# lightbulb128/troy

Measured on AMD Instinct MI355X. Metric: ct x ct multiply+relinearize ops/sec, BFV N=2^15 L=14; achieved HBM GB/s vs peak, higher is better.
Workload: dtype u64; 1 GPU; bfv_n32768_l14; scheme=BFV, N=32768, K=15, L=14, batch_per_gpu=256, parallelism=batch-shard x1, streams_per_gpu=2, Bsk=15, limb_transforms_per_op=443

## Files before the change

### troy_amd/csrc/device_types.h

```cpp
#pragma once
#include "modarith.h"

namespace troyhip {

struct PrimeDesc {
    u64 p, cr0, cr1, two_p;
    Shoup inv_n;
    Shoup iroot_last_scaled;
    Shoup r64;
    const Shoup *root;
    const Shoup *iroot;
    Shoup aux;
    const Shoup *root_fp;
    const Shoup *iroot_fp;
    Shoup inv_n_fp, iroot_last_scaled_fp;
    const u64 *root_w;
    const u64 *iroot_w;
};
__host__ __device__ inline Mod mod_of(const PrimeDesc &d) { return Mod{d.p, d.cr0, d.cr1}; }

struct LimbMap {
    uint8_t id[64];
    uint32_t period, inner;
    uint64_t lean;
    uint64_t fp;
    const uint64_t *host_primes;
};

#define TROY_BUF_OOB 0x80000000u
#ifdef TROYHIP_CPU_EMUL
#define TROY_WAVE_SYNC() hip_emul::park(2)
#define TROY_DYN_LDS(type, name) static type name[160 * 1024 / sizeof(type)]
#define TROY_GLDS16(gptr, lds_base) memcpy((char *)(lds_base) + 16 * (threadIdx.x & 63), (const void *)(gptr), 16)
#define TROY_GLDS16_POL(gptr, lds_base, pol) TROY_GLDS16(gptr, lds_base)
struct MfmaFrag { int8_t bytes[16]; };
struct MfmaAcc { int32_t v[16]; };
#define TROY_MFMA_I8(fa, fb, fc) hip_emul::mfma_i32_32x32x32_i8((fa).bytes, (fb).bytes, (fc).v)
inline void frag_set_word(MfmaFrag &f, int pos, u64 v) { memcpy(f.bytes + 8 * pos, &v, 8); }
struct BufRsrc { char *base; u32 bytes; };
inline BufRsrc make_rsrc(const void *p, u32 bytes) { return BufRsrc{(char *)p, bytes}; }
inline u64 buf_load_u64(BufRsrc r, u32 off) { u64 v = 0; if ((u64)off + 8 <= r.bytes) memcpy(&v, r.base + off, 8); return v; }
inline void buf_store_u64(BufRsrc r, u32 off, u64 v) { if ((u64)off + 8 <= r.bytes) memcpy(r.base + off, &v, 8); }
#define TROY_WAIT_VMEM() hip_emul::park(2)
#define TROY_WAIT_LDS() hip_emul::park(2)
#else
struct MfmaFrag { int bytes __attribute__((ext_vector_type(4))); };
struct MfmaAcc { int v __attribute__((ext_vector_type(16))); };
#define TROY_MFMA_I8(fa, fb, fc) ((fc).v = __builtin_amdgcn_mfma_i32_32x32x32_i8((fa).bytes, (fb).bytes, (fc).v, 0, 0, 0))
__device__ __forceinline__ void frag_set_word(MfmaFrag &f, int pos, u64 v) {
    f.bytes[2 * pos] = (int)(u32)v;
    f.bytes[2 * pos + 1] = (int)(u32)(v >> 32);
}
typedef __amdgpu_buffer_rsrc_t BufRsrc;
typedef unsigned int troy_v2u __attribute__((ext_vector_type(2)));
__device__ __forceinline__ BufRsrc make_rsrc(const void *p, u32 bytes) { return __builtin_amdgcn_make_buffer_rsrc((void *)p, 0, (int)bytes, 0x00020000); }
__device__ __forceinline__ u64 buf_load_u64(BufRsrc r, u32 off) {
    const troy_v2u v = __builtin_amdgcn_raw_buffer_load_b64(r, (int)off, 0, 0);
    return (u64)v.x | ((u64)v.y << 32);
}
__device__ __forceinline__ void buf_store_u64(BufRsrc r, u32 off, u64 v) {
    troy_v2u d;
    d.x = (u32)v;
    d.y = (u32)(v >> 32);
    __builtin_amdgcn_raw_buffer_store_b64(d, r, (int)off, 0, 0);
}
#define TROY_GLDS16(gptr, lds_base)                                                                                      \
    __builtin_amdgcn_global_load_lds((const __attribute__((address_space(1))) void *)(gptr), (__attribute__((address_space(3))) void *)(lds_base), 16, 0, 0)
#define TROY_GLDS16_POL(gptr, lds_base, pol)                                                                             \
    __builtin_amdgcn_global_load_lds((const __attribute__((address_space(1))) void *)(gptr), (__attribute__((address_space(3))) void *)(lds_base), 16, 0, pol)
#define TROY_WAIT_VMEM() asm volatile("s_waitcnt vmcnt(0)" ::: "memory")
#define TROY_WAIT_LDS() asm volatile("s_waitcnt lgkmcnt(0)" ::: "memory")
#define TROY_WAVE_SYNC() __builtin_amdgcn_wave_barrier()
#define TROY_DYN_LDS(type, name) extern __shared__ __attribute__((aligned(16))) type name[]
#endif

}
```

### troy_amd/csrc/ntt2.hip

```cpp
#include "kernels.h"
#include "bfly.h"
#include "fpmod.h"
#include <cstdio>
#include <cstdlib>
#include <cstring>
#include <type_traits>

namespace troyhip {

#define N2_THREADS 256
#define N2_LOGT 11
#define N2_T 2048

struct Ntt2Args {
    u64 *data;
    const u64 *src;
    u64 src_ostride;
    const PrimeDesc *primes;
    LimbMap map;
    int logn;
    unsigned tiles_per_row_log;
    unsigned m_total;
    unsigned rows_per_wg;
    unsigned chunks;
// ... 127 lines not shown
            for (int st = 0; st < R; st++) {
                const int dist = 1 << st, off = (1 << R) - ((1 << R) >> st);
                const bool last = STRIDED && (LS + st == NS - 1);
#pragma unroll
                for (int u = 0; u < G; u++)
#pragma unroll
                    for (int blk = 0; blk < ((1 << R) >> (st + 1)); blk++)
#pragma unroll
                        for (int k = 0; k < dist; k++) {
                            const int ix = (u << R) + blk * 2 * dist + k, iy = ix + dist;
                            const Shoup &w = tw[u][off + blk];
                            const double X = fp_of_bits(x[ix]), Y = fp_of_bits(x[iy]);
                            const double sum = X + Y, dif = X - Y;
                            x[ix] = fp_bits(last ? fp_mulmod_wp(sum, fp_of_bits(inv_n.op), fp_of_bits(inv_n.quo), fc) : sum);
                            x[iy] = fp_bits(fp_mulmod_wp(dif, fp_of_bits(w.op), fp_of_bits(w.quo), fc));
                        }
            }
            return;
        }
#pragma unroll
        for (int st = 0; st < R; st++) {
#pragma unroll
            for (int u = 0; u < G; u++) {
                const int half = (1 << R) >> (st + 1);
#pragma unroll
                for (int blk = 0; blk < (1 << st); blk++)
#pragma unroll
                    for (int k = 0; k < half; k++) {
                        const int ix = (u << R) + blk * 2 * half + k, iy = ix + half;
                        const Shoup &w = tw[u][(1 << st) - 1 + blk];
                        const double X = fp_of_bits(x[ix]);
                        const double v = fp_mulmod_wp(fp_of_bits(x[iy]), fp_of_bits(w.op), fp_of_bits(w.quo), fc);
                        x[ix] = fp_bits(X + v);
                        x[iy] = fp_bits(X - v);
                    }
            }
        }
    }
    __device__ static __forceinline__ void compute(u64 (&x)[8], const Shoup (&tw)[G][NTW], const PrimeDesc &pd, const bool lean = false) {
        const PrimeConst pc = make_prime_const(pd.p);
#pragma unroll
        for (int st = 0; st < R; st++) {
            u64 X[4], Y[4];
            Shoup w[4];
            int ix[4], iy[4];
            int n = 0;
#pragma unroll
            for (int u = 0; u < G; u++) {
                if (!INV) {
                    const int half = (1 << R) >> (st + 1);
#pragma unroll
                    for (int blk = 0; blk < (1 << st); blk++)
#pragma unroll
                        for (int k = 0; k < half; k++) {
                            ix[n] = (u << R) + blk * 2 * half + k;
                            iy[n] = ix[n] + half;
                            w[n] = tw[u][(1 << st) - 1 + blk];
                            n++;
                        }
                } else {
                    const int dist = 1 << st;
                    const int off = (1 << R) - ((1 << R) >> st);
#pragma unroll
                    for (int blk = 0; blk < ((1 << R) >> (st + 1)); blk++)
#pragma unroll
                        for (int k = 0; k < dist; k++) {
                            ix[n] = (u << R) + blk * 2 * dist + k;
                            iy[n] = ix[n] + dist;
                            w[n] = tw[u][off + blk];
                            n++;
                        }
                }
            }
#pragma unroll
            for (int i = 0; i < 4; i++) { X[i] = x[ix[i]]; Y[i] = x[iy[i]]; }
            if (!INV) {
                if (lean) ct_bfly4_ng<UNIFORM>(X, Y, w, pc); else ct_bfly4<UNIFORM>(X, Y, w, pc);
            } else if (STRIDED && (LS + st == NS - 1)) gs_bfly4_last<UNIFORM>(X, Y, w, pd.inv_n, pc);
            else gs_bfly4<UNIFORM>(X, Y, w, pc);
#pragma unroll
            for (int i = 0; i < 4; i++) { x[ix[i]] = X[i]; x[iy[i]] = Y[i]; }
        }
    }
    __device__ static __forceinline__ void lds_read(u64 (&x)[8], const u64 *lds, const unsigned t) {
#pragma unroll
        for (int u = 0; u < G; u++)
#pragma unroll
            for (int e = 0; e < (1 << R); e++) x[(u << R) + e] = lds[swz(elem(t + THREADS * u, e))];
    }
    __device__ static __forceinline__ void lds_write(const u64 (&x)[8], u64 *lds, const unsigned t) {
#pragma unroll
        for (int u = 0; u < G; u++)
#pragma unroll
            for (int e = 0; e < (1 << R); e++) lds[swz(elem(t + THREADS * u, e))] = x[(u << R) + e];
    }
    __device__ static __forceinline__ unsigned unit_perm(unsigned lane) { return 4 * (lane & 15) + (lane >> 4); }
    __device__ static __forceinline__ void stage_issue(const u64 *row, unsigned tile, u64 *wave_stage) {
        static_assert(!STRIDED && NS == 9 && R == 3 && LS == 0, "staging is defined for the first round of the contiguous pass");
        const unsigned lane = threadIdx.x & 63, w = threadIdx.x >> 6;
        const u64 *src = row + ((size_t)tile << N2_LOGT) + 512 * w + 2 * (INV ? unit_perm(lane) : lane);
#pragma unroll
        for (int i = 0; i < 4; i++) TROY_GLDS16_POL(src + 128 * i, wave_stage + 128 * i, 2);
    }
    __device__ static __forceinline__ void stage_read(u64 (&x)[8], const u64 *wave_stage) {
        const unsigned lane = threadIdx.x & 63;
        if (INV) {
            const u64 *mine = wave_stage + 128 * (lane >> 4) + 2 * (lane & 15);
#pragma unroll
            for (int j = 0; j < 4; j++) {
                const ulonglong2 v = *reinterpret_cast<const ulonglong2 *>(mine + 32 * j);
                x[2 * j] = v.x;
                x[2 * j + 1] = v.y;
            }
        } else {
#pragma unroll
            for (int e = 0; e < 8; e++) x[e] = wave_stage[lane + 64 * e];
        }
    }
    __device__ static __forceinline__ void store_via_lds(const u64 (&x)[8], u64 *row, unsigned tile, u64 *wave_xchg) {
        const unsigned lane = threadIdx.x & 63, w = threadIdx.x >> 6;
        u64 *mine = wave_xchg + 128 * (lane >> 4) + 2 * (lane & 15);
#pragma unroll
        for (int j = 0; j < 4; j++) {
            ulonglong2 v;
            v.x = x[2 * j];
            v.y = x[2 * j + 1];
            *reinterpret_cast<ulonglong2 *>(mine + 32 * j) = v;
        }
        TROY_WAVE_SYNC();
        u64 *dst = row + ((size_t)tile << N2_LOGT) + 512 * w + 2 * unit_perm(lane);
#pragma unroll
        for (int c = 0; c < 4; c++) {
            const ulonglong2 v = *reinterpret_cast<const ulonglong2 *>(wave_xchg + 128 * c + 2 * lane);
            *reinterpret_cast<ulonglong2 *>(dst + 128 * c) = v;
        }
    }
    __device__ static __forceinline__ void tensor_epilogue(u64 (&x)[8], u64 (&tx)[3][8], unsigned mm, u64 *out, unsigned period, unsigned slot, unsigned tile, int logn,
                                                           const Mod &m, u64 *xchg, const bool lean, const FpPrime *fc = nullptr) {
        const PrimeConst pc = make_prime_const(m.p);
        if (fc) {
#pragma unroll
            for (int e = 0; e < 8; e++) x[e] = fp_canonical(fp_of_bits(x[e]), *fc, m.p);
        } else if (lean) {
#pragma unroll
            for (int h = 0; h < 2; h++) {
                u64 v[4] = {x[4 * h], x[4 * h + 1], x[4 * h + 2], x[4 * h + 3]};
                lite_reduce4(v, (u32)m.cr1, pc);
#pragma unroll
                for (int i = 0; i < 4; i++) x[4 * h + i] = v[i];
            }
        } else {
#pragma unroll
            for (int h = 0; h < 2; h++) {
                u64 v[4] = {x[4 * h], x[4 * h + 1], x[4 * h + 2], x[4 * h + 3]};
                reduce4_from_8p(v, pc);
#pragma unroll
                for (int i = 0; i < 4; i++) x[4 * h + i] = v[i];
            }
        }
        const unsigned vr = mm & 3;
        if (vr < 3) {
#pragma unroll
            for (int i = 0; i < 3; i++)
                if ((int)vr == i) {
#pragma unroll
                    for (int e = 0; e < 8; e++) tx[i][e] = x[e];
                }
            return;
        }
        const unsigned b = mm >> 2;
        const ProdMod pm = make_prod_mod(m);
        u64 d[3][8];
#pragma unroll
        for (int e = 0; e < 8; e++) {
            const u64 a0 = tx[0][e], a1 = tx[1][e], b0 = tx[2][e], b1 = x[e];
            d[0][e] = reduce_prod((u128)a0 * b0, pm);
            d[1][e] = reduce_prod((u128)a0 * b1 + (u128)a1 * b0, pm);
// ... 72 lines not shown
                    v.x = x[(u << R) + e];
                    v.y = x[(u << R) + e + 1];
                    *reinterpret_cast<ulonglong2 *>(row + g_index<STRIDED, NS, LOGC>(tile, elem(q, e), logn)) = v;
                }
            } else {
#pragma unroll
                for (int e = 0; e < (1 << R); e++) n2_st<STRIDED && !INV>(row + g_index<STRIDED, NS, LOGC>(tile, elem(q, e), logn), x[(u << R) + e]);
            }
        }
    }
    template <int FINAL> __device__ static __forceinline__ void md_write(u64 (&x)[8], const Ntt2Args &a, unsigned o, unsigned slot, unsigned tile, int logn, const Mod &m,
                                                                         const PrimeDesc &pd, const FpPrime *fc = nullptr) {
        static_assert(INV && STRIDED && G == 1, "the mod-down epilogue belongs to the last inverse pass");
        const u64 p = m.p;
        const PrimeConst pc = make_prime_const(p);
        const u64 *sp = a.data + (((u64)o * a.map.period + a.md_dl) << logn);
        u64 *ct = a.md_ct + (u64)(o >> 1) * a.md_ct_bstride + (((u64)(o & 1) * a.md_dl + slot) << logn);
        const u64 *base = a.md_base ? a.md_base + (u64)(o >> 1) * a.md_base_bstride + (((u64)(o & 1) * a.md_dl + slot) << logn) : ct;
        const bool from_zero = a.md_base && (o & 1) && a.md_base_polys < 2;
        const ulonglong2 *sh = reinterpret_cast<const ulonglong2 *>(a.md_share) + ((u64)o << logn);
        const u64 c_p = FINAL == 3 ? barrett64(a.md_half, m) : 0;
#pragma unroll
        for (int h = 0; h < 2; h++) {
            u64 v[4] = {x[4 * h], x[4 * h + 1], x[4 * h + 2], x[4 * h + 3]};
            if (fc) {
#pragma unroll
                for (int i = 0; i < 4; i++) v[i] = fp_canonical(fp_of_bits(v[i]), *fc, p);
            } else {
                reduce4_from_4p(v, pc);
            }
            u64 al[4], ah[4], c[4];
            unsigned n[4];
#pragma unroll
            for (int i = 0; i < 4; i++) {
                n[i] = g_index<STRIDED, NS, LOGC>(tile, elem(threadIdx.x, 4 * h + i), logn);
                if (FINAL == 3) { al[i] = sp[n[i]]; ah[i] = 0; }
                else { const ulonglong2 t = sh[n[i]]; al[i] = t.x; ah[i] = t.y; }
                c[i] = from_zero ? 0 : base[n[i]];
            }
#pragma unroll
            for (int i = 0; i < 4; i++) {
                u64 w;
                if (FINAL == 3) {
                    u64 tl = al[i] + a.md_half;
                    tl = tl >= a.md_qk ? tl - a.md_qk : tl;
                    w = p + c_p - barrett64(tl, m);
                } else {
                    w = p - barrett128(al[i], ah[i], m);
                }
                u64 r = v[i] + mul_shoup(w, pd.aux, p);
                r = r >= p ? r - p : r;
                ct[n[i]] = addmod(c[i], r, p);
            }
        }
    }
};

template <int NS> struct Plan;
template <> struct Plan<3> { static constexpr int r[4] = {3, 0, 0, 0}; };
template <> struct Plan<4> { static constexpr int r[4] = {3, 1, 0, 0}; };
template <> struct Plan<5> { static constexpr int r[4] = {3, 2, 0, 0}; };
template <> struct Plan<6> { static constexpr int r[4] = {3, 3, 0, 0}; };
template <> struct Plan<7> { static constexpr int r[4] = {3, 1, 3, 0}; };
template <> struct Plan<9> { static constexpr int r[4] = {3, 3, 3, 0}; };
template <> struct Plan<10> { static constexpr int r[4] = {3, 3, 3, 1}; };
template <> struct Plan<11> { static constexpr int r[4] = {3, 3, 3, 2}; };

template <int INV, int STRIDED, int NS, int LOGC, int FINAL, int REDUCE, int MAC, int FP>
__device__ __forceinline__ void ntt2_body(const Ntt2Args &a) {
    static_assert(!FP || !(INV && MAC), "FP64 instances: every pass of the two-pass transform and its fusions");
    constexpr int LOGT = STRIDED ? NS + LOGC : N2_LOGT;
    __shared__ u64 lds[2][1 << LOGT];
    using P = Plan<NS>;
    constexpr bool WAVE_PRIVATE = !STRIDED && NS == 9;
    constexpr bool KS = MAC == 1 || MAC == 3;
    constexpr int FRESH = (!STRIDED && !INV && NS == 9 && MAC == 0) ? (FINAL ? 15 : 1)
                          : (STRIDED && !INV && NS == 7)                 ? 1
                          : (!STRIDED && NS == 10)                       ? 63
                          : (FINAL >= 3 && NS >= 6)                      ? 15
                          : MAC == 2                                     ? 15
                          : (FP && MAC)                                  ? 15
                          : (STRIDED && !INV && !REDUCE && NS >= 4 && NS <= 6) ? 15
                                                                         : 0;
    auto round_sync = [&]() {
        if (WAVE_PRIVATE) TROY_WAVE_SYNC(); else __syncthreads();
    };
    constexpr int R0 = P::r[0], R1 = P::r[1], R2 = P::r[2], R3 = P::r[3];
    constexpr int NR = (R0 > 0) + (R1 > 0) + (R2 > 0) + (R3 > 0);
    constexpr int Q0 = INV ? P::r[NR - 1] : R0;
    constexpr int Q1 = NR > 1 ? (INV ? P::r[NR - 2] : R1) : 0;
    constexpr int Q2 = NR > 2 ? (INV ? P::r[NR - 3] : R2) : 0;
    constexpr int Q3 = NR > 3 ? (INV ? P::r[NR - 4] : R3) : 0;
    using Rd0 = Round<INV, STRIDED, NS, LOGC, 0, Q0>;
    using Rd1 = Round<INV, STRIDED, NS, LOGC, Q0, Q1 ? Q1 : 1>;
    using Rd2 = Round<INV, STRIDED, NS, LOGC, Q0 + Q1, Q2 ? Q2 : 1>;
    using Rd3 = Round<INV, STRIDED, NS, LOGC, Q0 + Q1 + Q2, Q3 ? Q3 : 1>;

    const unsigned tile = blockIdx.x & ((1u << a.tiles_per_row_log) - 1);
    const unsigned grp = blockIdx.x >> a.tiles_per_row_log;
    const unsigned sidx = a.slot_fastest ? grp % a.nsel : grp / a.chunks, chunk = a.slot_fastest ? grp / a.nsel : grp % a.chunks;
    const unsigned slot = (unsigned)__builtin_amdgcn_readfirstlane((int)a.sel[sidx]);
    PrimeDesc pd = a.primes[a.map.id[slot]];
    if constexpr (FP) { pd.root = pd.root_fp; pd.iroot = pd.iroot_fp; pd.inv_n = pd.inv_n_fp; pd.iroot_last_scaled = pd.iroot_last_scaled_fp; }
    const FpPrime fc_ = make_fp_prime_uniform(FP ? pd.p : 1);
    const FpPrime &fc = fc_;
    const FpPrime *const fcp = FP ? &fc_ : nullptr;
    const Mod m = mod_of(pd);
    const bool need_reduce = !FP && REDUCE && (a.src_bound == 0 || (pd.p >> 61) != 0 || a.src_bound > 8 * pd.p);
    const bool lean = !INV && ((a.map.lean >> slot) & 1);
    const int logn = a.logn;
    const int k1 = STRIDED ? NS : logn - NS;
    const int s_first = INV ? (STRIDED ? k1 - 1 : logn - 1) : (STRIDED ? 0 : k1);

    Shoup tw0[Rd0::G][Rd0::NTW], tw1[Rd1::G][Rd1::NTW], tw2[Rd2::G][Rd2::NTW], tw3[Rd3::G][Rd3::NTW];
    Rd0::load_tw(tw0, pd, tile, logn, s_first);
    if constexpr (NR > 1) Rd1::load_tw(tw1, pd, tile, logn, s_first);
    if constexpr (NR > 2) Rd2::load_tw(tw2, pd, tile, logn, s_first);
    if constexpr (NR > 3) Rd3::load_tw(tw3, pd, tile, logn, s_first);
    Rd0::settle_tw(tw0);
    if constexpr (NR > 1) Rd1::settle_tw(tw1);
    if constexpr (NR > 2) Rd2::settle_tw(tw2);
    if constexpr (NR > 3) Rd3::settle_tw(tw3);

    const unsigned m_begin = chunk * a.rows_per_wg;
    const unsigned m_end = (m_begin + a.rows_per_wg < a.m_total) ? m_begin + a.rows_per_wg : a.m_total;
    const unsigned inner = a.map.inner, period = a.map.period;
    auto fp_guard = [&](u64 (&v)[8], int r) {
        if constexpr (FP) {
            if ((a.fp_red_mask >> r) & 1) {
#pragma unroll
                for (int e = 0; e < 8; e++) v[e] = fp_bits(fp_reduce(fp_of_bits(v[e]), fc));
            }
        }
    };
    auto row_ptrs = [&](unsigned mm, unsigned o, unsigned k, u64 *&row, const u64 *&in) {
        if constexpr (MAC == 2) {
            const unsigned b = mm >> 2, vr = mm & 3;
            row = (vr < 2 ? a.data : a.tensor_b) + ((((u64)b * 2 + (vr & 1)) * period + slot) << logn);
            in = row;
            return;
        }
        const u64 r = ((u64)o * period + slot) * inner + k;
        row = a.data + (r << logn);
        in = (REDUCE || a.src) ? (a.src_same_layout ? a.src + (r << logn) : a.src + (u64)o * a.src_ostride + ((u64)k << logn)) : row;
        if constexpr (!REDUCE && STRIDED && !INV) {
            if (a.src_same_layout == 2)
                in = slot >= a.src_slots ? row : (o < a.src_split ? a.src + (((u64)o * a.src_slots + slot) << logn) : a.src2 + (((u64)(o - a.src_split) * a.src_slots + slot) << logn));
        }
    };
    constexpr bool DMA = WAVE_PRIVATE;
    static_assert(MAC != 3 || DMA, "the CKKS key-switch pass (MAC = 3) takes its rows from the LDS-DMA staging area");
    constexpr bool PF = STRIDED && !INV && NR == 2 && !REDUCE;
    u64 xn[PF ? 8 : 1];
    static_assert(!MAC || (!INV && !STRIDED && NS == 9), "the inner product is fused into the forward contiguous pass");
    u64 tx[MAC == 2 ? 3 : 1][8];
    Acc128 macc[2][2][4];
    if (KS) {
#pragma unroll
        for (int cpt = 0; cpt < 2; cpt++)
#pragma unroll
            for (int g = 0; g < 2; g++)
#pragma unroll
                for (int e = 0; e < 4; e++) macc[cpt][g][e] = Acc128{0, 0, 0, 0};
    }
    double facc[2][FP ? 8 : 1];
    if constexpr (FP) {
#pragma unroll
        for (int cpt = 0; cpt < 2; cpt++)
#pragma unroll
            for (int e = 0; e < 8; e++) facc[cpt][e] = 0.0;
    }
    auto mac_row = [&](const u64 (&xr)[8], const ulonglong2 (&kw)[2][KS ? 4 : 1], unsigned row_no) {
        if constexpr (FP && KS) {
#pragma unroll
            for (int cpt = 0; cpt < 2; cpt++)
#pragma unroll
                for (int e = 0; e < 8; e++) {
                    const u64 kword = (e & 1) ? kw[cpt][e >> 1].y : kw[cpt][e >> 1].x;
                    facc[cpt][e] += fp_mulmod_pinv(fp_of_bits(xr[e]), fp_from_u64(kword), fc);
                }
            if (a.fp_acc_every && (row_no + 1) % a.fp_acc_every == 0) {
#pragma unroll
                for (int cpt = 0; cpt < 2; cpt++)
#pragma unroll
                    for (int e = 0; e < 8; e++) facc[cpt][e] = fp_reduce(facc[cpt][e], fc);
            }
        } else if constexpr (KS) {
#pragma unroll
            for (int cpt = 0; cpt < 2; cpt++) {
#pragma unroll
                for (int g = 0; g < 2; g++) {
                    const ulonglong2 k01 = kw[cpt][2 * g], k23 = kw[cpt][2 * g + 1];
                    const u64 kk[4] = {k01.x, k01.y, k23.x, k23.y};
                    const u64 xx[4] = {xr[4 * g], xr[4 * g + 1], xr[4 * g + 2], xr[4 * g + 3]};
                    mac128x4(macc[cpt][g], xx, kk);
                }
            }
        }
        (void)row_no;
    };
    const unsigned key_limb = KS ? (unsigned)__builtin_amdgcn_readfirstlane((int)a.mac_key_limb[slot]) : 0;
    constexpr bool MAC_STORE_LINEAR = KS && WAVE_PRIVATE;
    u64 *const wave_stage = lds[1] + 512 * (threadIdx.x >> 6);
    u64 x[8];
    unsigned ro = m_begin / inner, rk = m_begin - ro * inner;
    unsigned parity = 0;
    auto is_diag = [&](unsigned k) { return (MAC == 3 || REDUCE == 2) && k == slot; };
    {
        u64 *row0; const u64 *in0;
        row_ptrs(m_begin, ro, rk, row0, in0);
        if (!is_diag(rk)) {
            if constexpr (DMA) Rd0::stage_issue(in0, tile, wave_stage);
            else Rd0::template g_read<REDUCE>(x, in0, tile, logn, m);
        }
    }
    for (unsigned mm = m_begin; mm < m_end; mm++) {
        u64 *row; const u64 *in;
        row_ptrs(mm, ro, rk, row, in);
        const unsigned no = rk + 1 == inner ? ro + 1 : ro, nk = rk + 1 == inner ? 0 : rk + 1;
        const bool next_wanted = mm + 1 < m_end && !is_diag(nk);
        const bool skip_row = REDUCE == 2 && is_diag(rk);
        if constexpr (DMA) TROY_WAIT_VMEM();
        ulonglong2 kv[2][KS ? 4 : 1];
        auto load_keys = [&]() {
            const unsigned kk = rk;
            const u64 *kp = a.mac_key + ((((u64)kk * 2) * a.mac_K + key_limb) << logn) + ((u64)tile << N2_LOGT) + 8 * threadIdx.x;
#pragma unroll
            for (int cpt = 0; cpt < 2; cpt++) {
                const ulonglong2 *kq = reinterpret_cast<const ulonglong2 *>(kp + ((u64)cpt * a.mac_K << logn));
#pragma unroll
                for (int e = 0; e < 4; e++) kv[cpt][KS ? e : 0] = kq[e];
            }
        };
        if constexpr (KS) load_keys();
        if constexpr (MAC == 3) {
            const bool diag = is_diag(rk);
            if (!diag) {
                Rd0::stage_read(x, wave_stage);
                TROY_WAIT_LDS();
            }
            if (next_wanted) {
                u64 *nrow; const u64 *nin;
                row_ptrs(mm + 1, no, nk, nrow, nin);
                Rd0::stage_issue(nin, tile, wave_stage);
            }
            if (!diag) {
                u64 *buf = lds[0];
                fp_guard(x, 0);
                if constexpr (FP) Rd0::compute_fp(x, tw0, fc, pd.inv_n); else Rd0::compute(x, tw0, pd, lean);
                Rd0::lds_write(x, buf, (FRESH & 1) ? n2_opaque(threadIdx.x) : threadIdx.x);
                round_sync();
                Rd1::lds_read(x, buf, (FRESH & 2) ? n2_opaque(threadIdx.x) : threadIdx.x);
                fp_guard(x, 1);
                if constexpr (FP) Rd1::compute_fp(x, tw1, fc, pd.inv_n); else Rd1::compute(x, tw1, pd, lean);
                Rd1::lds_write(x, buf, (FRESH & 4) ? n2_opaque(threadIdx.x) : threadIdx.x);
                round_sync();
                Rd2::lds_read(x, buf, (FRESH & 8) ? n2_opaque(threadIdx.x) : threadIdx.x);
                fp_guard(x, 2);
                if constexpr (FP) Rd2::compute_fp(x, tw2, fc, pd.inv_n); else Rd2::compute(x, tw2, pd, lean);
                if constexpr (FP) {
                } else if (!a.mac_lazy && lean) {
#pragma unroll
                    for (int e = 0; e < 8; e++) x[e] = barrett64(x[e], m);
                } else if (!a.mac_lazy) {
                    const PrimeConst pc = make_prime_const(pd.p);
#pragma unroll
                    for (int h = 0; h < 2; h++) {
                        u64 v[4] = {x[4 * h], x[4 * h + 1], x[4 * h + 2], x[4 * h + 3]};
                        reduce4_from_8p(v, pc);
#pragma unroll
                        for (int i = 0; i < 4; i++) x[4 * h + i] = v[i];
                    }
                }
            } else {
                const ulonglong2 *tp = reinterpret_cast<const ulonglong2 *>(a.mac_target + (u64)ro * a.mac_tstride + ((u64)rk << logn) + ((u64)tile << N2_LOGT) + 8 * threadIdx.x);
#pragma unroll
                for (int e = 0; e < 4; e++) { const ulonglong2 v = tp[e]; x[2 * e] = v.x; x[2 * e + 1] = v.y; }
                if constexpr (FP) {
#pragma unroll
                    for (int e = 0; e < 8; e++) x[e] = fp_bits(fp_from_u64(x[e]));
                }
            }
            mac_row(x, kv, mm - m_begin);
            ro = no;
            rk = nk;
            continue;
        }
        if constexpr (DMA) {
            Rd0::stage_read(x, wave_stage);
            TROY_WAIT_LDS();
            if (next_wanted) {
                u64 *nrow; const u64 *nin;
                row_ptrs(mm + 1, no, nk, nrow, nin);
                Rd0::stage_issue(nin, tile, wave_stage);
            }
        }
        if (!skip_row) {
        u64 *buf = DMA ? lds[0] : lds[parity];
        if (REDUCE && need_reduce) {
#pragma unroll
            for (int e = 0; e < 8; e++) x[e] = barrett64(x[e], m);
        }
        if constexpr (FP && REDUCE) {
            if ((a.fp_src_wide >> rk) & 1) {
#pragma unroll
                for (int e = 0; e < 8; e++) x[e] = barrett64(x[e], m);
            }
#pragma unroll
            for (int e = 0; e < 8; e++) x[e] = fp_bits(fp_from_u64(x[e]));
        } else if constexpr (FP && ((!INV && STRIDED) || (INV && !STRIDED))) {
#pragma unroll
            for (int e = 0; e < 8; e++) x[e] = fp_bits(fp_from_u64(x[e]));
        }
        fp_guard(x, 0);
        if constexpr (FP) Rd0::compute_fp(x, tw0, fc, pd.inv_n); else Rd0::compute(x, tw0, pd, lean);
        if constexpr (NR == 1) {
            if constexpr (FINAL >= 3) Rd0::template md_write<FINAL>(x, a, mm, slot, tile, logn, m, pd, fcp);
            else Rd0::template g_write<FINAL>(x, row, tile, logn, m, lean, nullptr, fcp);
        } else {
            Rd0::lds_write(x, buf, (FRESH & 1) ? n2_opaque(threadIdx.x) : threadIdx.x);
            round_sync();
            Rd1::lds_read(x, buf, (FRESH & 2) ? n2_opaque(threadIdx.x) : threadIdx.x);
            if constexpr (PF) {
                if (mm + 1 < m_end) {
                    u64 *nrow; const u64 *nin;
                    row_ptrs(mm + 1, no, nk, nrow, nin);
                    Rd0::template g_read<REDUCE>(xn, nin, tile, logn, m, n2_opaque(threadIdx.x));
                }
            }
            fp_guard(x, 1);
            if constexpr (FP) Rd1::compute_fp(x, tw1, fc, pd.inv_n); else Rd1::compute(x, tw1, pd, lean);
            if constexpr (NR == 2) {
                if constexpr (FINAL >= 3) Rd1::template md_write<FINAL>(x, a, mm, slot, tile, logn, m, pd, fcp);
                else Rd1::template g_write<FINAL>(x, row, tile, logn, m, lean, nullptr, fcp);
            } else {
                Rd1::lds_write(x, buf, (FRESH & 4) ? n2_opaque(threadIdx.x) : threadIdx.x);
                round_sync();
                Rd2::lds_read(x, buf, (FRESH & 8) ? n2_opaque(threadIdx.x) : threadIdx.x);
                fp_guard(x, 2);
                if constexpr (FP) Rd2::compute_fp(x, tw2, fc, pd.inv_n); else Rd2::compute(x, tw2, pd, lean);
                if constexpr (NR == 3 && MAC == 2) {
                    Rd2::tensor_epilogue(x, tx, mm, a.tensor_out, period, slot, tile, logn, m, WAVE_PRIVATE ? buf : nullptr, lean, fcp);
                } else if constexpr (NR == 3 && KS) {
                    if constexpr (FP) {
                    } else if (!a.mac_lazy && lean) {
#pragma unroll
                        for (int e = 0; e < 8; e++) x[e] = barrett64(x[e], m);
                    } else if (!a.mac_lazy) {
                        const PrimeConst pc = make_prime_const(pd.p);
#pragma unroll
                        for (int h = 0; h < 2; h++) {
                            u64 v[4] = {x[4 * h], x[4 * h + 1], x[4 * h + 2], x[4 * h + 3]};
                            reduce4_from_8p(v, pc);
#pragma unroll
                            for (int i = 0; i < 4; i++) x[4 * h + i] = v[i];
                        }
                    }
                        mac_row(x, kv, mm - m_begin);
                } else if constexpr (NR == 3) {
                    if constexpr (FINAL >= 3) Rd2::template md_write<FINAL>(x, a, mm, slot, tile, logn, m, pd, fcp);
                    else Rd2::template g_write<FINAL>(x, row, tile, logn, m, lean, WAVE_PRIVATE ? buf : nullptr, fcp);
                } else {
                    Rd2::lds_write(x, buf, (FRESH & 16) ? n2_opaque(threadIdx.x) : threadIdx.x);
                    round_sync();
                    Rd3::lds_read(x, buf, (FRESH & 32) ? n2_opaque(threadIdx.x) : threadIdx.x);
                    fp_guard(x, 3);
                    if constexpr (FP) Rd3::compute_fp(x, tw3, fc, pd.inv_n); else Rd3::compute(x, tw3, pd, lean);
                    Rd3::template g_write<FINAL>(x, row, tile, logn, m, lean, nullptr, fcp);
                }
            }
        }
        }
        if constexpr (PF) {
#pragma unroll
            for (int e = 0; e < 8; e++) x[e] = xn[PF ? e : 0];
        } else if constexpr (!DMA) {
            if (next_wanted) {
                u64 *nrow; const u64 *nin;
                row_ptrs(mm + 1, no, nk, nrow, nin);
                if constexpr (FINAL >= 3) Rd0::template g_read<REDUCE>(x, nin, tile, logn, m, n2_opaque(threadIdx.x));
                else Rd0::template g_read<REDUCE>(x, nin, tile, logn, m);
            }
        }
        ro = no;
        rk = nk;
        if (!skip_row) parity ^= 1u;
    }
    if constexpr (KS) {
        const unsigned o = m_begin / inner;
        const u64 pos = ((u64)tile << N2_LOGT) + 8 * threadIdx.x;
#pragma unroll
        for (int cpt = 0; cpt < 2; cpt++) {
            ulonglong2 *op = reinterpret_cast<ulonglong2 *>(a.mac_acc + ((((u64)o * 2 + cpt) * period + slot) << logn) + pos);
            u64 lin[8];
#pragma unroll
            for (int e = 0; e < 4; e++) {
                ulonglong2 v;
                if constexpr (FP) {
                    v.x = fp_canonical(facc[cpt][2 * e], fc, m.p);
                    v.y = fp_canonical(facc[cpt][2 * e + 1], fc, m.p);
                } else {
                    const Acc128 &p0 = macc[cpt][e >> 1][2 * (e & 1)], &p1 = macc[cpt][e >> 1][2 * (e & 1) + 1];
                    v.x = barrett128(mk64(p0.a0, p0.a1), mk64(p0.a2, p0.a3), m);
                    v.y = barrett128(mk64(p1.a0, p1.a1), mk64(p1.a2, p1.a3), m);
                }
                if constexpr (MAC_STORE_LINEAR) { lin[2 * e] = v.x; lin[2 * e + 1] = v.y; }
                else op[e] = v;
            }
            if constexpr (MAC_STORE_LINEAR) {
                TROY_WAVE_SYNC();
                Rd2::store_via_lds(lin, a.mac_acc + ((((u64)o * 2 + cpt) * period + slot) << logn), tile, lds[0] + 512 * (threadIdx.x >> 6));
            }
            (void)lin;
        }
    }
}

template <int INV, int STRIDED, int NS, int LOGC, int FINAL, int REDUCE, int MAC = 0>
__global__ __launch_bounds__(STRIDED ? (1 << (NS + LOGC - 3)) : N2_THREADS, MAC == 2 ? 3 : MAC ? 2 : 4) void ntt2_kernel(Ntt2Args a) {
    ntt2_body<INV, STRIDED, NS, LOGC, FINAL, REDUCE, MAC, 0>(a);
}
template <int INV, int STRIDED, int NS, int LOGC, int FINAL, int REDUCE, int MAC = 0>
__global__ __launch_bounds__(STRIDED ? (1 << (NS + LOGC - 3)) : N2_THREADS, MAC ? 3 : 4) void ntt2_fp_kernel(Ntt2Args a) {
    ntt2_body<INV, STRIDED, NS, LOGC, FINAL, REDUCE, MAC, 1>(a);
}

bool ntt2_supported(int logn) { return logn >= 12 && logn <= 17; }

#ifndef TROYHIP_CPU_EMUL
#define N2_KTAG(...) do { if (ktime::enabled) { static thread_local char tagbuf[112]; std::snprintf(tagbuf, sizeof(tagbuf), __VA_ARGS__); ktime::tag = tagbuf; } } while (0)
#else
#define N2_KTAG(...)
#endif
static bool n2_wide(unsigned narrow_blocks) {
    static const int forced = [] { const char *e = probe_env("TROYHIP_NTT2_WIDE"); return e ? std::atoi(e) : -1; }();
    if (forced >= 0) return forced != 0;
    return (narrow_blocks >> 1) >= 4u * device_cus();
}
template <int INV, int STRIDED, int NS, int LOGC, int FINAL, int REDUCE> static void launch_one(const Ntt2Args &a, unsigned blocks, hipStream_t s, bool fp = false) {
    constexpr unsigned THREADS = STRIDED ? (1u << (NS + LOGC - 3)) : N2_THREADS;
    if (fp) {
        N2_KTAG("ntt2_fp_kernel<%d, %d, %d, %d, %d, %d, 0>", INV, STRIDED, NS, LOGC, FINAL, REDUCE);
        TROY_LAUNCH(HIP_KERNEL_NAME(ntt2_fp_kernel<INV, STRIDED, NS, LOGC, FINAL, REDUCE>), dim3(blocks), dim3(THREADS), 0, s, a);
        launch_check("ntt2_fp_kernel");
        return;
    }
    N2_KTAG("ntt2_kernel<%d, %d, %d, %d, %d, %d, 0>", INV, STRIDED, NS, LOGC, FINAL, REDUCE);
    TROY_LAUNCH(HIP_KERNEL_NAME(ntt2_kernel<INV, STRIDED, NS, LOGC, FINAL, REDUCE>), dim3(blocks), dim3(THREADS), 0, s, a);
    launch_check("ntt2_kernel");
}
template <int INV, int NS> static void launch_contig(const Ntt2Args &a, unsigned blocks, bool final_pass, hipStream_t s, bool fp = false) {
    if (final_pass) launch_one<INV, 0, NS, 0, INV ? 2 : 1, 0>(a, blocks, s, fp);
    else launch_one<INV, 0, NS, 0, 0, 0>(a, blocks, s, fp);
}
template <int INV, int NS> static void launch_strided(const Ntt2Args &a, unsigned blocks, bool final_pass, bool reduce, hipStream_t s, int md_kind = -1, bool skip_diag = false,
                                                      bool fp = false) {
    constexpr int LOGC = N2_LOGT - NS;
    if (INV) {
        if (md_kind == 0) launch_one<1, 1, NS, LOGC, 3, 0>(a, blocks, s, fp);
        else if (md_kind == 2) launch_one<1, 1, NS, LOGC, 4, 0>(a, blocks, s, fp);
        else launch_one<1, 1, NS, LOGC, 2, 0>(a, blocks, s, fp);
    } else {
        (void)final_pass;
        if constexpr (NS == 6) {
            if (!reduce && n2_wide(blocks)) {
                Ntt2Args w = a;
                w.tiles_per_row_log = a.tiles_per_row_log - 1;
                stats::counter(stats::NTT2_WIDE_LAUNCHES).fetch_add(1, std::memory_order_relaxed);
                launch_one<0, 1, NS, LOGC + 1, 0, 0>(w, blocks >> 1, s, fp);
                return;
            }
        }
        if (reduce && skip_diag) launch_one<0, 1, NS, LOGC, 0, 2>(a, blocks, s, fp);
        else if (reduce) launch_one<0, 1, NS, LOGC, 0, 1>(a, blocks, s, fp);
        else launch_one<0, 1, NS, LOGC, 0, 0>(a, blocks, s, fp);
    }
}
static int pass_rounds(int ns, bool inverse, int (&out)[4]) {
    const int *r = nullptr;
    switch (ns) {
    case 3: r = Plan<3>::r; break;
    case 4: r = Plan<4>::r; break;
    case 5: r = Plan<5>::r; break;
    case 6: r = Plan<6>::r; break;
    case 7: r = Plan<7>::r; break;
    case 9: r = Plan<9>::r; break;
    case 10: r = Plan<10>::r; break;
    default: r = Plan<11>::r; break;
    }
    int n = 0;
    for (int i = 0; i < 4; i++) if (r[i]) n++;
    for (int i = 0; i < n; i++) out[i] = inverse ? r[n - 1 - i] : r[i];
    return n;
}
static unsigned select_class(const LimbMap &map, unsigned slot_begin, unsigned slot_count, bool fp, uint8_t (&sel)[64]) {
    unsigned n = 0;
    for (unsigned i = slot_begin; i < slot_begin + slot_count; i++)
        if ((bool)((map.fp >> i) & 1) == fp) sel[n++] = (uint8_t)i;
    return n;
}

void launch_ntt2(u64 *data, const u64 *src, u64 src_ostride, bool src_reduce, const PrimeDesc *primes, const LimbMap &map, size_t rows, int logn,
                 bool inverse, hipStream_t stream, bool src_same_layout, u64 src_bound) {
    launch_ntt2_slots(data, src, src_ostride, src_reduce, primes, map, rows, logn, inverse, stream, src_same_layout, src_bound, 0, map.period, nullptr);
}
void launch_ntt2_slots(u64 *data, const u64 *src, u64 src_ostride, bool src_reduce, const PrimeDesc *primes, const LimbMap &map, size_t rows, int logn,
                       bool inverse, hipStream_t stream, bool src_same_layout, u64 src_bound, unsigned slot_begin, unsigned slot_count, const Ntt2ModDown *md,
                       unsigned passes, unsigned plan_begin, unsigned plan_count) {
    const u64 *host_primes = map.host_primes;
    if (plan_count && plan_begin + plan_count > map.period) throw Error(ST_INVALID_ARGUMENT, "ntt2: plan slot range");
    if (rows == 0 || slot_count == 0) return;
    if (slot_begin + slot_count > map.period) throw Error(ST_INVALID_ARGUMENT, "ntt2: slot range");
    const bool partial = slot_begin != 0 || slot_count != map.period;
    if ((partial || md || passes != 3) && (!inverse || src)) throw Error(ST_LOGIC_ERROR, "ntt2: slot ranges, single passes and the mod-down epilogue belong to the in-place inverse transform");
    if (md && !(passes & 2)) throw Error(ST_LOGIC_ERROR, "ntt2: the mod-down epilogue rides on the second pass");
    if (md && map.inner != 1) throw Error(ST_LOGIC_ERROR, "ntt2: the mod-down epilogue takes one row per (item, prime)");
    if (!ntt2_supported(logn)) throw Error(ST_LOGIC_ERROR, "ntt2: unsupported size");
    const size_t per_outer = (size_t)map.period * map.inner;
    if (rows % per_outer) throw Error(ST_INVALID_ARGUMENT, "ntt2: row count must be a multiple of the limb pattern");
    if (src && inverse) throw Error(ST_LOGIC_ERROR, "ntt2: out-of-place input is only supported by the forward transform");
// ... 160 lines not shown
        second.mac_lazy = lazy;
        std::memcpy(second.mac_key_limb, key_limb, map.period);
        if (fp) {
            N2_KTAG("ntt2_fp_kernel<0, 0, 9, 0, 1, 0, %d>", skip_diag ? 3 : 1);
            if (skip_diag) TROY_LAUNCH(HIP_KERNEL_NAME(ntt2_fp_kernel<0, 0, 9, 0, 1, 0, 3>), dim3(blocks), dim3(N2_THREADS), 0, stream, second);
            else TROY_LAUNCH(HIP_KERNEL_NAME(ntt2_fp_kernel<0, 0, 9, 0, 1, 0, 1>), dim3(blocks), dim3(N2_THREADS), 0, stream, second);
        } else if (skip_diag) {
            N2_KTAG("ntt2_kernel<0, 0, 9, 0, 1, 0, 3>");
            TROY_LAUNCH(HIP_KERNEL_NAME(ntt2_kernel<0, 0, 9, 0, 1, 0, 3>), dim3(blocks), dim3(N2_THREADS), 0, stream, second);
        } else {
            N2_KTAG("ntt2_kernel<0, 0, 9, 0, 1, 0, 1>");
            TROY_LAUNCH(HIP_KERNEL_NAME(ntt2_kernel<0, 0, 9, 0, 1, 0, 1>), dim3(blocks), dim3(N2_THREADS), 0, stream, second);
        }
        launch_check("ntt2_kernel(ks_mac)");
    }
}

bool ntt2_tensor_supported(int logn) { return ntt2_supported(logn) && logn - 9 >= 3 && logn - 9 <= 7; }
bool ntt2_ks_mac_supported(int logn) { return ntt2_tensor_supported(logn); }
void launch_ntt2_tensor(u64 *xa, const u64 *src_a, u64 *xb, const u64 *src_b, u64 *out, const PrimeDesc *primes, const LimbMap &map, size_t batch, int logn,
                        hipStream_t stream, unsigned src_slots) {
    const u64 *host_primes = map.host_primes;
    if (!batch) return;
    if (!ntt2_tensor_supported(logn) || map.inner != 1) throw Error(ST_LOGIC_ERROR, "ntt2 tensor: unsupported shape");
    const int k1 = logn - 9;
    const bool same = xa == xb;
    const bool joint = src_slots && !same && xb == xa + ((batch * 2 * map.period) << logn);
    if (src_slots && (!src_a || !src_b || src_slots > map.period)) throw Error(ST_LOGIC_ERROR, "ntt2 tensor: operands of the merged form");
    for (int cls = 0; cls < 2; cls++) {
        const bool fp = cls == 1;
        if (fp && !host_primes) break;
        uint8_t sel[64];
        unsigned nsel = 0;
        if (host_primes) nsel = select_class(map, 0, map.period, fp, sel);
        else for (unsigned i = 0; i < map.period; i++) sel[nsel++] = (uint8_t)i;
        if (!nsel) continue;
        stats::counter(fp ? stats::NTT2_FP_LAUNCHES : stats::NTT2_INT_LAUNCHES).fetch_add(1, std::memory_order_relaxed);
        unsigned mask1 = 0, mask2 = 0;
        if (fp) {
            u64 pmax = 0;
            for (unsigned i = 0; i < nsel; i++) pmax = std::max(pmax, host_primes[map.id[sel[i]]]);
            int r1[4], r2[4];
            const int n1 = pass_rounds(k1, false, r1), n2 = pass_rounds(9, false, r2);
            const FpPlan p1 = fp_plan(pmax, 1.0, r1, n1), p2 = fp_plan(pmax, p1.out_bound, r2, n2);
            mask1 = p1.mask; mask2 = p2.mask;
        }
        for (int part = 0; part < (same || joint ? 1 : 2); part++) {
            Ntt2Args a;
            std::memset(&a, 0, sizeof(a));
            a.data = part ? xb : xa;
            const u64 *src = part ? src_b : src_a;
            a.primes = primes;
            a.map = map;
            a.logn = logn;
            a.tiles_per_row_log = (unsigned)(logn - N2_LOGT);
            a.m_total = (unsigned)(batch * (joint ? 4 : 2));
            a.nsel = nsel;
            std::memcpy(a.sel, sel, sizeof(sel));
            a.fp_red_mask = mask1;
            a.rows_per_wg = plan_per_workgroup(a.m_total, a.m_total < 8 ? a.m_total : 8, (size_t)nsel << a.tiles_per_row_log);
            a.chunks = (a.m_total + a.rows_per_wg - 1) / a.rows_per_wg;
            if (src_slots) { a.src = src; a.src2 = src_b; a.src_same_layout = 2; a.src_slots = src_slots; a.src_split = joint ? (unsigned)(batch * 2) : ~0u; }
            else if (src) { a.src = src; a.src_same_layout = 1; }
            const unsigned blocks = (unsigned)((nsel * a.chunks) << a.tiles_per_row_log);
            switch (k1) {
            case 3: launch_strided<0, 3>(a, blocks, false, false, stream, -1, false, fp); break;
            case 4: launch_strided<0, 4>(a, blocks, false, false, stream, -1, false, fp); break;
            case 5: launch_strided<0, 5>(a, blocks, false, false, stream, -1, false, fp); break;
            case 6: launch_strided<0, 6>(a, blocks, false, false, stream, -1, false, fp); break;
            default: launch_strided<0, 7>(a, blocks, false, false, stream, -1, false, fp); break;
            }
        }
        Ntt2Args a;
        std::memset(&a, 0, sizeof(a));
        a.data = xa; a.tensor_b = xb; a.tensor_out = out;
        a.primes = primes;
        a.map = map;
        a.logn = logn;
        a.tiles_per_row_log = (unsigned)(logn - N2_LOGT);
        a.m_total = (unsigned)(batch * 4);
        a.nsel = nsel;
        std::memcpy(a.sel, sel, sizeof(sel));
        a.fp_red_mask = mask2;
        a.rows_per_wg = 4;
        a.chunks = (unsigned)batch;
        const unsigned blocks = (unsigned)((nsel * a.chunks) << a.tiles_per_row_log);
        if (fp) {
            N2_KTAG("ntt2_fp_kernel<0, 0, 9, 0, 1, 0, 2>");
            TROY_LAUNCH(HIP_KERNEL_NAME(ntt2_fp_kernel<0, 0, 9, 0, 1, 0, 2>), dim3(blocks), dim3(N2_THREADS), 0, stream, a);
        } else {
            N2_KTAG("ntt2_kernel<0, 0, 9, 0, 1, 0, 2>");
            TROY_LAUNCH(HIP_KERNEL_NAME(ntt2_kernel<0, 0, 9, 0, 1, 0, 2>), dim3(blocks), dim3(N2_THREADS), 0, stream, a);
        }
        launch_check("ntt2_kernel(tensor)");
    }
}

}
```

### troy_amd/csrc/rt.h

```cpp
#pragma once

#include <atomic>
#include <cstddef>
#include <cstdint>
#include <cstdlib>
#include <stdexcept>
#include <string>

#ifdef TROYHIP_CPU_EMUL
#include "hip_emul.h"
#else
#include <hip/hip_runtime.h>
#include <atomic>
namespace troyhip { namespace ktime {
extern std::atomic<bool> enabled;
extern thread_local const char *tag;
void begin(const char *name, hipStream_t s);
void end(hipStream_t s);
} }
#define TROY_LAUNCH(kernel, grid, block, shmem, stream, ...)                          \
    do {                                                                              \
        const dim3 troy_grid_ = dim3(grid);                                           \
        if (!troy_grid_.x || !troy_grid_.y || !troy_grid_.z) break;                   \
        if (::troyhip::ktime::enabled) ::troyhip::ktime::begin(#kernel, stream);      \
        kernel<<<troy_grid_, block, shmem, stream>>>(__VA_ARGS__);                    \
        if (::troyhip::ktime::enabled) ::troyhip::ktime::end(stream);                 \
    } while (0)
#endif

namespace troyhip {

inline const char *probe_env(const char *name) {
#ifdef TROYHIP_PROBES
    return std::getenv(name);
#else
    (void)name;
    return nullptr;
#endif
}

namespace stats {
enum { KS_FP_LAUNCHES, KS_INT_LAUNCHES, NTT1_FP_LAUNCHES, NTT1_INT_LAUNCHES, NTT2_FP_LAUNCHES, NTT2_INT_LAUNCHES, BEHZ_FP_LAUNCHES, BEHZ_MFMA_LAUNCHES, BEHZ_VALU_LAUNCHES, NTT2_WIDE_LAUNCHES, ENC_TAIL_ITEMS, COUNT };
inline std::atomic<uint64_t> &counter(int i) { static std::atomic<uint64_t> c[COUNT]; return c[i]; }
inline const char *name(int i) { static const char *n[COUNT] = {"ks_fp_launches", "ks_int_launches", "ntt1_fp_launches", "ntt1_int_launches", "ntt2_fp_launches", "ntt2_int_launches", "behz_fp_launches", "behz_mfma_launches", "behz_valu_launches", "ntt2_wide_launches", "enc_tail_items"}; return n[i]; }
}

typedef uint64_t u64;
typedef uint32_t u32;
typedef unsigned __int128 u128;

struct Error : std::runtime_error {
    int code;
    Error(int c, const std::string &m) : std::runtime_error(m), code(c) {}
};

enum { ST_OK = 0, ST_INVALID_ARGUMENT = 1, ST_LOGIC_ERROR = 2, ST_OUT_OF_RANGE = 3, ST_RUNTIME_ERROR = 4, ST_NOT_INITIALIZED = 5 };

inline void hip_check(hipError_t e, const char *what) {
    if (e != hipSuccess) throw Error(ST_RUNTIME_ERROR, std::string("HIP error: ") + hipGetErrorString(e) + " in " + what);
}
#define HIP_CHECK(x) ::troyhip::hip_check((x), #x)

inline void launch_check(const char *name) {
    hipError_t e = hipGetLastError();
    if (e != hipSuccess) throw Error(ST_RUNTIME_ERROR, std::string("kernel launch failed: ") + name + ": " + hipGetErrorString(e));
}

inline unsigned ceil_div(size_t a, size_t b) { return (unsigned)((a + b - 1) / b); }

}
```

Before: 9713 ops/s.

## Group tensor-product rows per workgroup and refine NTT2 LDS addressing and waits

The tensor-product NTT2 launch now packs several batch items into each workgroup (up to four), choosing the group count from the CU count so twiddle loads and setup are amortized over more rows. Twiddle loading for wave-private kernels is deferred until after the initial prefetch so it overlaps with memory traffic. The MAC path uses a partial vmcnt wait to keep later loads in flight, and MAC kernels use an XOR-based LDS address computation that hoists the base swizzle. The cost is fewer workgroups, which can reduce occupancy and load balance for small batches, and the partial wait depends on the load count assumed by the code.

New measurement: 9762 ops/s, median of 6. Within noise of the previous version (+0.5%).

```diff
diff --git a/troy_amd/csrc/device_types.h b/troy_amd/csrc/device_types.h
--- a/troy_amd/csrc/device_types.h
+++ b/troy_amd/csrc/device_types.h
@@ -42,6 +42,7 @@
 inline u64 buf_load_u64(BufRsrc r, u32 off) { u64 v = 0; if ((u64)off + 8 <= r.bytes) memcpy(&v, r.base + off, 8); return v; }
 inline void buf_store_u64(BufRsrc r, u32 off, u64 v) { if ((u64)off + 8 <= r.bytes) memcpy(r.base + off, &v, 8); }
 #define TROY_WAIT_VMEM() hip_emul::park(2)
+#define TROY_WAIT_VMEM_KEEP(n) hip_emul::park(2)
 #define TROY_WAIT_LDS() hip_emul::park(2)
 #else
 struct MfmaFrag { int bytes __attribute__((ext_vector_type(4))); };
@@ -69,6 +70,7 @@
 #define TROY_GLDS16_POL(gptr, lds_base, pol)                                                                             \
     __builtin_amdgcn_global_load_lds((const __attribute__((address_space(1))) void *)(gptr), (__attribute__((address_space(3))) void *)(lds_base), 16, 0, pol)
 #define TROY_WAIT_VMEM() asm volatile("s_waitcnt vmcnt(0)" ::: "memory")
+#define TROY_WAIT_VMEM_KEEP(n) asm volatile("s_waitcnt vmcnt(" #n ")" ::: "memory")
 #define TROY_WAIT_LDS() asm volatile("s_waitcnt lgkmcnt(0)" ::: "memory")
 #define TROY_WAVE_SYNC() __builtin_amdgcn_wave_barrier()
 #define TROY_DYN_LDS(type, name) extern __shared__ __attribute__((aligned(16))) type name[]
diff --git a/troy_amd/csrc/ntt2.hip b/troy_amd/csrc/ntt2.hip
--- a/troy_amd/csrc/ntt2.hip
+++ b/troy_amd/csrc/ntt2.hip
@@ -233,17 +233,27 @@
             for (int i = 0; i < 4; i++) { x[ix[i]] = X[i]; x[iy[i]] = Y[i]; }
         }
     }
-    __device__ static __forceinline__ void lds_read(u64 (&x)[8], const u64 *lds, const unsigned t) {
-#pragma unroll
-        for (int u = 0; u < G; u++)
-#pragma unroll
-            for (int e = 0; e < (1 << R); e++) x[(u << R) + e] = lds[swz(elem(t + THREADS * u, e))];
-    }
-    __device__ static __forceinline__ void lds_write(const u64 (&x)[8], u64 *lds, const unsigned t) {
-#pragma unroll
-        for (int u = 0; u < G; u++)
-#pragma unroll
-            for (int e = 0; e < (1 << R); e++) lds[swz(elem(t + THREADS * u, e))] = x[(u << R) + e];
+    template <bool XF = false> __device__ static __forceinline__ void lds_read(u64 (&x)[8], const u64 *lds, const unsigned t) {
+#pragma unroll
+        for (int u = 0; u < G; u++) {
+            const unsigned b8 = swz(base_of(t + THREADS * u)) << 3;
+#pragma unroll
+            for (int e = 0; e < (1 << R); e++) {
+                if constexpr (XF) x[(u << R) + e] = *reinterpret_cast<const u64 *>(reinterpret_cast<const char *>(lds) + (b8 ^ (swz((unsigned)e << LOGD) << 3)));
+                else x[(u << R) + e] = lds[swz(elem(t + THREADS * u, e))];
+            }
+        }
+    }
+    template <bool XF = false> __device__ static __forceinline__ void lds_write(const u64 (&x)[8], u64 *lds, const unsigned t) {
+#pragma unroll
+        for (int u = 0; u < G; u++) {
+            const unsigned b8 = swz(base_of(t + THREADS * u)) << 3;
+#pragma unroll
+            for (int e = 0; e < (1 << R); e++) {
+                if constexpr (XF) *reinterpret_cast<u64 *>(reinterpret_cast<char *>(lds) + (b8 ^ (swz((unsigned)e << LOGD) << 3))) = x[(u << R) + e];
+                else lds[swz(elem(t + THREADS * u, e))] = x[(u << R) + e];
+            }
+        }
     }
     __device__ static __forceinline__ unsigned unit_perm(unsigned lane) { return 4 * (lane & 15) + (lane >> 4); }
     __device__ static __forceinline__ void stage_issue(const u64 *row, unsigned tile, u64 *wave_stage) {
@@ -482,6 +492,7 @@
                           : (FP && MAC)                                  ? 15
                           : (STRIDED && !INV && !REDUCE && NS >= 4 && NS <= 6) ? 15
                                                                          : 0;
+    constexpr bool XF = MAC != 0 && FRESH != 0;
     auto round_sync = [&]() {
         if (WAVE_PRIVATE) TROY_WAVE_SYNC(); else __syncthreads();
     };
@@ -513,14 +524,17 @@
     const int s_first = INV ? (STRIDED ? k1 - 1 : logn - 1) : (STRIDED ? 0 : k1);
 
     Shoup tw0[Rd0::G][Rd0::NTW], tw1[Rd1::G][Rd1::NTW], tw2[Rd2::G][Rd2::NTW], tw3[Rd3::G][Rd3::NTW];
-    Rd0::load_tw(tw0, pd, tile, logn, s_first);
-    if constexpr (NR > 1) Rd1::load_tw(tw1, pd, tile, logn, s_first);
-    if constexpr (NR > 2) Rd2::load_tw(tw2, pd, tile, logn, s_first);
-    if constexpr (NR > 3) Rd3::load_tw(tw3, pd, tile, logn, s_first);
-    Rd0::settle_tw(tw0);
-    if constexpr (NR > 1) Rd1::settle_tw(tw1);
-    if constexpr (NR > 2) Rd2::settle_tw(tw2);
-    if constexpr (NR > 3) Rd3::settle_tw(tw3);
+    auto load_twiddles = [&]() {
+        Rd0::load_tw(tw0, pd, tile, logn, s_first);
+        if constexpr (NR > 1) Rd1::load_tw(tw1, pd, tile, logn, s_first);
+        if constexpr (NR > 2) Rd2::load_tw(tw2, pd, tile, logn, s_first);
+        if constexpr (NR > 3) Rd3::load_tw(tw3, pd, tile, logn, s_first);
+        Rd0::settle_tw(tw0);
+        if constexpr (NR > 1) Rd1::settle_tw(tw1);
+        if constexpr (NR > 2) Rd2::settle_tw(tw2);
+        if constexpr (NR > 3) Rd3::settle_tw(tw3);
+    };
+    if constexpr (!WAVE_PRIVATE) load_twiddles();
 
     const unsigned m_begin = chunk * a.rows_per_wg;
     const unsigned m_end = (m_begin + a.rows_per_wg < a.m_total) ? m_begin + a.rows_per_wg : a.m_total;
@@ -614,13 +628,16 @@
             else Rd0::template g_read<REDUCE>(x, in0, tile, logn, m);
         }
     }
+    if constexpr (WAVE_PRIVATE) load_twiddles();
     for (unsigned mm = m_begin; mm < m_end; mm++) {
         u64 *row; const u64 *in;
         row_ptrs(mm, ro, rk, row, in);
         const unsigned no = rk + 1 == inner ? ro + 1 : ro, nk = rk + 1 == inner ? 0 : rk + 1;
         const bool next_wanted = mm + 1 < m_end && !is_diag(nk);
         const bool skip_row = REDUCE == 2 && is_diag(rk);
-        if constexpr (DMA) TROY_WAIT_VMEM();
+        if constexpr (MAC == 2) {
+            if ((mm & 3) == 0 && mm != m_begin) TROY_WAIT_VMEM_KEEP(12); else TROY_WAIT_VMEM();
+        } else if constexpr (DMA) TROY_WAIT_VMEM();
         ulonglong2 kv[2][KS ? 4 : 1];
         auto load_keys = [&]() {
             const unsigned kk = rk;
@@ -648,14 +665,14 @@
                 u64 *buf = lds[0];
                 fp_guard(x, 0);
                 if constexpr (FP) Rd0::compute_fp(x, tw0, fc, pd.inv_n); else Rd0::compute(x, tw0, pd, lean);
-                Rd0::lds_write(x, buf, (FRESH & 1) ? n2_opaque(threadIdx.x) : threadIdx.x);
+                Rd0::template lds_write<XF>(x, buf, (FRESH & 1) ? n2_opaque(threadIdx.x) : threadIdx.x);
                 round_sync();
-                Rd1::lds_read(x, buf, (FRESH & 2) ? n2_opaque(threadIdx.x) : threadIdx.x);
+                Rd1::template lds_read<XF>(x, buf, (FRESH & 2) ? n2_opaque(threadIdx.x) : threadIdx.x);
                 fp_guard(x, 1);
                 if constexpr (FP) Rd1::compute_fp(x, tw1, fc, pd.inv_n); else Rd1::compute(x, tw1, pd, lean);
-                Rd1::lds_write(x, buf, (FRESH & 4) ? n2_opaque(threadIdx.x) : threadIdx.x);
+                Rd1::template lds_write<XF>(x, buf, (FRESH & 4) ? n2_opaque(threadIdx.x) : threadIdx.x);
                 round_sync();
-                Rd2::lds_read(x, buf, (FRESH & 8) ? n2_opaque(threadIdx.x) : threadIdx.x);
+                Rd2::template lds_read<XF>(x, buf, (FRESH & 8) ? n2_opaque(threadIdx.x) : threadIdx.x);
                 fp_guard(x, 2);
                 if constexpr (FP) Rd2::compute_fp(x, tw2, fc, pd.inv_n); else Rd2::compute(x, tw2, pd, lean);
                 if constexpr (FP) {
@@ -718,9 +735,9 @@
             if constexpr (FINAL >= 3) Rd0::template md_write<FINAL>(x, a, mm, slot, tile, logn, m, pd, fcp);
             else Rd0::template g_write<FINAL>(x, row, tile, logn, m, lean, nullptr, fcp);
         } else {
-            Rd0::lds_write(x, buf, (FRESH & 1) ? n2_opaque(threadIdx.x) : threadIdx.x);
+            Rd0::template lds_write<XF>(x, buf, (FRESH & 1) ? n2_opaque(threadIdx.x) : threadIdx.x);
             round_sync();
-            Rd1::lds_read(x, buf, (FRESH & 2) ? n2_opaque(threadIdx.x) : threadIdx.x);
+            Rd1::template lds_read<XF>(x, buf, (FRESH & 2) ? n2_opaque(threadIdx.x) : threadIdx.x);
             if constexpr (PF) {
                 if (mm + 1 < m_end) {
                     u64 *nrow; const u64 *nin;
@@ -734,9 +751,9 @@
                 if constexpr (FINAL >= 3) Rd1::template md_write<FINAL>(x, a, mm, slot, tile, logn, m, pd, fcp);
                 else Rd1::template g_write<FINAL>(x, row, tile, logn, m, lean, nullptr, fcp);
             } else {
-                Rd1::lds_write(x, buf, (FRESH & 4) ? n2_opaque(threadIdx.x) : threadIdx.x);
+                Rd1::template lds_write<XF>(x, buf, (FRESH & 4) ? n2_opaque(threadIdx.x) : threadIdx.x);
                 round_sync();
-                Rd2::lds_read(x, buf, (FRESH & 8) ? n2_opaque(threadIdx.x) : threadIdx.x);
+                Rd2::template lds_read<XF>(x, buf, (FRESH & 8) ? n2_opaque(threadIdx.x) : threadIdx.x);
                 fp_guard(x, 2);
                 if constexpr (FP) Rd2::compute_fp(x, tw2, fc, pd.inv_n); else Rd2::compute(x, tw2, pd, lean);
                 if constexpr (NR == 3 && MAC == 2) {
@@ -836,6 +853,16 @@
     static const int forced = [] { const char *e = probe_env("TROYHIP_NTT2_WIDE"); return e ? std::atoi(e) : -1; }();
     if (forced >= 0) return forced != 0;
     return (narrow_blocks >> 1) >= 4u * device_cus();
+}
+#define N2_TENSOR_GMAX 4
+#define N2_TENSOR_ROUNDS 8
+static unsigned n2_tensor_groups(size_t batch, size_t wgs_per_item) {
+    static const int forced = [] { const char *e = probe_env("TROYHIP_TENSOR_GROUPS"); return e ? std::atoi(e) : 0; }();
+    if (forced > 0) return (unsigned)forced;
+    const size_t want = (size_t)N2_TENSOR_ROUNDS * 3 * device_cus();
+    unsigned g = N2_TENSOR_GMAX;
+    while (g > 1 && ((batch + g - 1) / g) * wgs_per_item < want) g >>= 1;
+    return g;
 }
 template <int INV, int STRIDED, int NS, int LOGC, int FINAL, int REDUCE> static void launch_one(const Ntt2Args &a, unsigned blocks, hipStream_t s, bool fp = false) {
     constexpr unsigned THREADS = STRIDED ? (1u << (NS + LOGC - 3)) : N2_THREADS;
@@ -1162,8 +1189,11 @@
         a.nsel = nsel;
         std::memcpy(a.sel, sel, sizeof(sel));
         a.fp_red_mask = mask2;
-        a.rows_per_wg = 4;
-        a.chunks = (unsigned)batch;
+        const unsigned groups = n2_tensor_groups(batch, (size_t)nsel << a.tiles_per_row_log);
+        stats::counter(stats::TENSOR_LAUNCHES).fetch_add(1, std::memory_order_relaxed);
+        stats::counter(stats::TENSOR_GROUP_SUM).fetch_add(groups, std::memory_order_relaxed);
+        a.rows_per_wg = 4 * groups;
+        a.chunks = (unsigned)((batch + groups - 1) / groups);
         const unsigned blocks = (unsigned)((nsel * a.chunks) << a.tiles_per_row_log);
         if (fp) {
             N2_KTAG("ntt2_fp_kernel<0, 0, 9, 0, 1, 0, 2>");
diff --git a/troy_amd/csrc/rt.h b/troy_amd/csrc/rt.h
--- a/troy_amd/csrc/rt.h
+++ b/troy_amd/csrc/rt.h
@@ -40,9 +40,9 @@
 }
 
 namespace stats {
-enum { KS_FP_LAUNCHES, KS_INT_LAUNCHES, NTT1_FP_LAUNCHES, NTT1_INT_LAUNCHES, NTT2_FP_LAUNCHES, NTT2_INT_LAUNCHES, BEHZ_FP_LAUNCHES, BEHZ_MFMA_LAUNCHES, BEHZ_VALU_LAUNCHES, NTT2_WIDE_LAUNCHES, ENC_TAIL_ITEMS, COUNT };
+enum { KS_FP_LAUNCHES, KS_INT_LAUNCHES, NTT1_FP_LAUNCHES, NTT1_INT_LAUNCHES, NTT2_FP_LAUNCHES, NTT2_INT_LAUNCHES, BEHZ_FP_LAUNCHES, BEHZ_MFMA_LAUNCHES, BEHZ_VALU_LAUNCHES, NTT2_WIDE_LAUNCHES, ENC_TAIL_ITEMS, TENSOR_LAUNCHES, TENSOR_GROUP_SUM, COUNT };
 inline std::atomic<uint64_t> &counter(int i) { static std::atomic<uint64_t> c[COUNT]; return c[i]; }
-inline const char *name(int i) { static const char *n[COUNT] = {"ks_fp_launches", "ks_int_launches", "ntt1_fp_launches", "ntt1_int_launches", "ntt2_fp_launches", "ntt2_int_launches", "behz_fp_launches", "behz_mfma_launches", "behz_valu_launches", "ntt2_wide_launches", "enc_tail_items"}; return n[i]; }
+inline const char *name(int i) { static const char *n[COUNT] = {"ks_fp_launches", "ks_int_launches", "ntt1_fp_launches", "ntt1_int_launches", "ntt2_fp_launches", "ntt2_int_launches", "behz_fp_launches", "behz_mfma_launches", "behz_valu_launches", "ntt2_wide_launches", "enc_tail_items", "tensor_launches", "tensor_group_sum"}; return n[i]; }
 }
 
 typedef uint64_t u64;
```
